# AlonKellner/hifi-gan

Measured on NVIDIA B200. Metric: V1 audio samples/sec, higher is better.
Workload: dtype bf16

## Files before the change

### hifi-gan_b200/csrc/hg_common.cuh

```cuda
#pragma once

#include <cuda_runtime.h>
#include <cuda_bf16.h>
#include <cuda.h>
#include <stdint.h>
#include <stdio.h>

#define HG_OK 0
#define HG_ERR_INVALID (-1)
#define HG_ERR_CUDA (-2)
#define HG_ERR_UNSUPPORTED (-3)
#define HG_ERR_DRIVER (-4)

void hg_set_error(const char* fmt, ...);

#define HG_CHECK_CUDA(expr)                                                        \
  do {                                                                             \
    cudaError_t _e = (expr);                                                       \
    if (_e != cudaSuccess) {                                                       \
      hg_set_error("%s:%d: %s -> %s", __FILE__, __LINE__, #expr,                   \
                   cudaGetErrorString(_e));                                        \
      return HG_ERR_CUDA;                                                          \
    }                                                                              \
  } while (0)
// ... 54 lines not shown
      "selp.b32 %0, 1, 0, P;\n\t"
      "}\n"
      : "=r"(ok)
      : "r"(smem_u32(bar)), "r"(parity)
      : "memory");
  return ok != 0;
}
__device__ __forceinline__ void mbar_wait(uint64_t* bar, uint32_t parity) {
  uint32_t spins = 0;
  while (!mbar_try_wait(bar, parity)) {
    if (++spins > HG_SPIN_LIMIT) {
      printf("hg: mbarrier wait timed out (block %d thread %d)\n", (int)blockIdx.x, (int)threadIdx.x);
      __trap();
    }
  }
}

__device__ __forceinline__ void tma_prefetch_desc(const CUtensorMap* m) {
  asm volatile("prefetch.tensormap [%0];" ::"l"(reinterpret_cast<uint64_t>(m)) : "memory");
}
__device__ __forceinline__ void tma_load_3d(void* smem_dst, const CUtensorMap* m, uint64_t* bar,
                                            int32_t c0, int32_t c1, int32_t c2) {
  asm volatile(
      "cp.async.bulk.tensor.3d.shared::cluster.global.mbarrier::complete_tx::bytes"
      " [%0], [%1, {%3, %4, %5}], [%2];"
      :
      : "r"(smem_u32(smem_dst)), "l"(reinterpret_cast<uint64_t>(m)), "r"(smem_u32(bar)), "r"(c0),
        "r"(c1), "r"(c2)
      : "memory");
}

__device__ __forceinline__ void tc_fence_before() {
  asm volatile("tcgen05.fence::before_thread_sync;" ::: "memory");
}
__device__ __forceinline__ void tc_fence_after() {
  asm volatile("tcgen05.fence::after_thread_sync;" ::: "memory");
}
__device__ __forceinline__ void tmem_alloc(uint32_t* smem_result, uint32_t ncols) {
  asm volatile("tcgen05.alloc.cta_group::1.sync.aligned.shared::cta.b32 [%0], %1;" ::"r"(
                   smem_u32(smem_result)),
               "r"(ncols)
               : "memory");
  asm volatile("tcgen05.relinquish_alloc_permit.cta_group::1.sync.aligned;" ::: "memory");
}
__device__ __forceinline__ void tmem_dealloc(uint32_t taddr, uint32_t ncols) {
  asm volatile("tcgen05.dealloc.cta_group::1.sync.aligned.b32 %0, %1;" ::"r"(taddr), "r"(ncols)
               : "memory");
}
__device__ __forceinline__ void umma_bf16_ss_lo(uint32_t d_tmem, uint32_t a_lo, uint32_t b_lo,
                                                uint32_t desc_hi, uint32_t idesc, uint32_t accumulate) {
  asm volatile(
      "{\n\t"
      ".reg .pred p;\n\t"
      ".reg .b64 da, db;\n\t"
      "setp.ne.b32 p, %5, 0;\n\t"
      "mov.b64 da, {%1, %3};\n\t"
      "mov.b64 db, {%2, %3};\n\t"
      "tcgen05.mma.cta_group::1.kind::f16 [%0], da, db, %4, p;\n\t"
      "}\n"
      :
      : "r"(d_tmem), "r"(a_lo), "r"(b_lo), "r"(desc_hi), "r"(idesc), "r"(accumulate)
      : "memory");
}
__device__ __forceinline__ uint32_t cluster_ctarank() {
  uint32_t r;
  asm volatile("mov.u32 %0, %%cluster_ctarank;" : "=r"(r));
  return r;
}
__device__ __forceinline__ void cluster_sync_all() {
  asm volatile("barrier.cluster.arrive.release.aligned;" ::: "memory");
  asm volatile("barrier.cluster.wait.acquire.aligned;" ::: "memory");
}
__device__ __forceinline__ void mbar_arrive_remote(uint64_t* bar, uint32_t cta) {
  asm volatile(
      "{\n\t"
      ".reg .b32 remAddr32;\n\t"
      "mapa.shared::cluster.u32 remAddr32, %0, %1;\n\t"
      "mbarrier.arrive.shared::cluster.b64 _, [remAddr32];\n\t"
      "}\n"
      :
      : "r"(smem_u32(bar)), "r"(cta)
      : "memory");
}
__device__ __forceinline__ void tma_load_3d_2sm(void* smem_dst, const CUtensorMap* m, uint64_t* bar,
                                                int32_t c0, int32_t c1, int32_t c2) {
  asm volatile(
      "cp.async.bulk.tensor.3d.cta_group::2.shared::cluster.global.mbarrier::complete_tx::bytes"
      " [%0], [%1, {%3, %4, %5}], [%2];"
      :
      : "r"(smem_u32(smem_dst)), "l"(reinterpret_cast<uint64_t>(m)), "r"(smem_u32(bar) & 0xFEFFFFFFu),
        "r"(c0), "r"(c1), "r"(c2)
      : "memory");
}
__device__ __forceinline__ void tmem_alloc_2sm(uint32_t* smem_result, uint32_t ncols) {
  asm volatile("tcgen05.alloc.cta_group::2.sync.aligned.shared::cta.b32 [%0], %1;" ::"r"(
                   smem_u32(smem_result)),
               "r"(ncols)
               : "memory");
  asm volatile("tcgen05.relinquish_alloc_permit.cta_group::2.sync.aligned;" ::: "memory");
}
__device__ __forceinline__ void tmem_dealloc_2sm(uint32_t taddr, uint32_t ncols) {
  asm volatile("tcgen05.dealloc.cta_group::2.sync.aligned.b32 %0, %1;" ::"r"(taddr), "r"(ncols)
               : "memory");
}
__device__ __forceinline__ void umma_bf16_ss_lo_2sm(uint32_t d_tmem, uint32_t a_lo, uint32_t b_lo,
                                                    uint32_t desc_hi, uint32_t idesc, uint32_t accumulate) {
  asm volatile(
      "{\n\t"
      ".reg .pred p;\n\t"
      ".reg .b64 da, db;\n\t"
      "setp.ne.b32 p, %5, 0;\n\t"
      "mov.b64 da, {%1, %3};\n\t"
      "mov.b64 db, {%2, %3};\n\t"
      "tcgen05.mma.cta_group::2.kind::f16 [%0], da, db, %4, p;\n\t"
      "}\n"
      :
      : "r"(d_tmem), "r"(a_lo), "r"(b_lo), "r"(desc_hi), "r"(idesc), "r"(accumulate)
      : "memory");
}
__device__ __forceinline__ void umma_commit_2sm(uint64_t* bar) {
  asm volatile(
      "tcgen05.commit.cta_group::2.mbarrier::arrive::one.shared::cluster.multicast::cluster.b64 [%0], %1;"
      :
      : "r"(smem_u32(bar)), "h"(static_cast<uint16_t>(3))
      : "memory");
}

__device__ __forceinline__ uint32_t umma_desc_lo(uint32_t saddr) {
  return ((saddr & 0x3FFFFu) >> 4) | (1u << 16);
}
__device__ __forceinline__ uint32_t umma_desc_hi(uint32_t sbo_bytes, uint32_t layout_type) {
  return ((sbo_bytes >> 4) & 0x3FFFu) | (1u << 14) | ((layout_type & 7u) << 29);
}
__device__ __forceinline__ void umma_commit(uint64_t* bar) {
  asm volatile("tcgen05.commit.cta_group::1.mbarrier::arrive::one.shared::cluster.b64 [%0];" ::"r"(
                   smem_u32(bar))
               : "memory");
}
__device__ __forceinline__ void tmem_ld_wait() {
  asm volatile("tcgen05.wait::ld.sync.aligned;" ::: "memory");
}


__host__ __device__ constexpr uint32_t umma_idesc_bf16(uint32_t M, uint32_t N) {
  return (1u << 4) | (1u << 7) | (1u << 10) | ((N >> 3) << 17) | ((M >> 4) << 24);
}

__device__ __forceinline__ float lrelu(float v, float slope) { return v > 0.f ? v : v * slope; }

__device__ __forceinline__ uint32_t pack_bf16x2(float lo, float hi) {
  __nv_bfloat162 h = __floats2bfloat162_rn(lo, hi);
  return *reinterpret_cast<uint32_t*>(&h);
}
__device__ __forceinline__ float2 unpack_bf16x2(uint32_t w) {
  __nv_bfloat162 h = *reinterpret_cast<__nv_bfloat162*>(&w);
  return __bfloat1622float2(h);
}

struct U8 {
  uint32_t v[8];
};

__device__ __forceinline__ U8 ldg256(const void* p) {
  U8 r;
  asm volatile("ld.global.nc.L1::no_allocate.v8.b32 {%0,%1,%2,%3,%4,%5,%6,%7}, [%8];"
               : "=r"(r.v[0]), "=r"(r.v[1]), "=r"(r.v[2]), "=r"(r.v[3]), "=r"(r.v[4]), "=r"(r.v[5]),
// ... 77 lines not shown
```

### hifi-gan_b200/csrc/hg_resblock_pair.cu

```cuda
#include "hg_common.cuh"

#include <atomic>

#include "../../include/hifigan_b200.h"

extern std::atomic<int64_t> g_hg_launches;

namespace {

constexpr int kM = 128;
constexpr int kXformWarps = 4;
__host__ __device__ constexpr int epi_halves(int c) { return c == 64 ? 2 : 1; }
__host__ __device__ constexpr int pair_threads(int c) { return 64 + (kXformWarps + 8 * epi_halves(c)) * 32; }
constexpr int kMaxXSlots = 4;

struct PairArgs {
  int batch, t, c;
  int ktaps, dil1;
  int single;
  int subs;
  int r_out;
  int pad1, pad2;
  int a_rows;
  int x_boxes, x_box_rows;
// ... 291 lines not shown
      }
      int i = 0, m = 0;
      for (int u = 0; u < n_units; ++u) {
        const uint32_t a = i & 1u, ph = (i >> 1) & 1u;
        off = off_next; valid = valid_next; keep = keep_next;
#pragma unroll
        for (int g = 0; g < kG; ++g) rcur[g] = rnext[g];
        if (u + 1 < n_units) {
          off_next = next_unit_off(valid_next, keep_next);
          if (valid_next) {
#pragma unroll
            for (int g = 0; g < kG; ++g) rnext[g] = hg::ldg256(p.x + off_next + g * 16);
          }
        }
        constexpr bool kPreRes = kMrf && (C == 32);
        hg::U8 r1[kPreRes ? kG : 1], r2[kPreRes ? kG : 1];
        if (kPreRes && valid && p.res1) {
#pragma unroll
          for (int g = 0; g < kG; ++g) r1[kPreRes ? g : 0] = hg::ldg256(p.res1 + off + g * 16);
        }
        if (kPreRes && valid && p.res2) {
#pragma unroll
          for (int g = 0; g < kG; ++g) r2[kPreRes ? g : 0] = hg::ldg256(p.res2 + off + g * 16);
        }
        if (m == 0) {
          hg::mbar_wait(&full_bar[a], ph);
          hg::tc_fence_after();
        }
#pragma unroll
        for (int g = 0; g < kG; ++g) {
          uint32_t raw[16];
          hg::tmem_ld_32x16(tmem_base + lane_base + acc_base + a * acc_cols + m * C + col0 + g * 16, raw);
          hg::tmem_ld_wait();
          if (g == kG - 1 && m == S - 1) {
            hg::tc_fence_before();
            __syncwarp();
            if (lane == 0) hg::mbar_arrive(&empty_bar[a]);
          }
          if (valid) {
            float v[16];
#pragma unroll
            for (int q = 0; q < 4; ++q) {
              const float4 bq = *reinterpret_cast<const float4*>(bias + col0 + g * 16 + 4 * q);
              v[4 * q] = __uint_as_float(raw[4 * q]) + bq.x;
              v[4 * q + 1] = __uint_as_float(raw[4 * q + 1]) + bq.y;
              v[4 * q + 2] = __uint_as_float(raw[4 * q + 2]) + bq.z;
              v[4 * q + 3] = __uint_as_float(raw[4 * q + 3]) + bq.w;
            }
            if (kActIn) hg::add_bf16x16_unlrelu(v, rcur[g], p.x_inv);
            else hg::add_bf16x16(v, rcur[g]);
            if (kMrf && p.res1) hg::add_bf16x16(v, kPreRes ? r1[kPreRes ? g : 0] : hg::ldg256(p.res1 + off + g * 16));
            if (kMrf && p.res2) hg::add_bf16x16(v, kPreRes ? r2[kPreRes ? g : 0] : hg::ldg256(p.res2 + off + g * 16));
            if (kMrf) {
              const float sc = keep ? p.scale : 0.f;
#pragma unroll
              for (int e = 0; e < 16; ++e) v[e] *= sc;
            }
            if (p.out_raw) {
              hg::U8 o;
#pragma unroll
              for (int q = 0; q < 8; ++q) o.v[q] = hg::pack_bf16x2(v[2 * q], v[2 * q + 1]);
              hg::stg256(p.out_raw + off + g * 16, o);
            }
            if (kMrf && p.out_act) {
              hg::U8 o;
#pragma unroll
              for (int q = 0; q < 8; ++q)
                o.v[q] = hg::pack_bf16x2(hg::lrelu(v[2 * q], p.out_slope), hg::lrelu(v[2 * q + 1], p.out_slope));
              hg::stg256(p.out_act + off + g * 16, o);
            }
          }
        }
        if (++m == S) { m = 0; ++i; }
      }
    }
  }

  hg::tc_fence_before();
  __syncthreads();
  hg::tc_fence_after();
  if (warp == 1) hg::tmem_dealloc(tmem_base, tmem_cols);
}

int g_sms = 0, g_smem = 0;

template <int C, bool kSingle, bool kMrf, bool kActIn>
int launch_pair_as(const CUtensorMap& tx, const CUtensorMap& tw1, const CUtensorMap& tw2, const PairArgs& p,
                size_t smem_bytes, int grid, cudaStream_t st) {
  static hg::PerDeviceOnce once;
  if (once.need())
    HG_CHECK_CUDA(cudaFuncSetAttribute(resblock_pair_kernel<C, kSingle, kMrf, kActIn>,
                                       cudaFuncAttributeMaxDynamicSharedMemorySize, g_smem));
  resblock_pair_kernel<C, kSingle, kMrf, kActIn><<<grid, pair_threads(C), smem_bytes, st>>>(tx, tw1, tw2, p);
  HG_CHECK_CUDA(cudaGetLastError());
  return HG_OK;
}

template <int C, bool kSingle>
int launch_pair(const CUtensorMap& tx, const CUtensorMap& tw1, const CUtensorMap& tw2, const PairArgs& p,
                bool act_in, size_t smem_bytes, int grid, cudaStream_t st) {
  const bool mrf = p.res1 || p.res2 || p.out_act || p.item_len || p.scale != 1.f;
  if (act_in)
    return mrf ? launch_pair_as<C, kSingle, true, true>(tx, tw1, tw2, p, smem_bytes, grid, st)
               : launch_pair_as<C, kSingle, false, true>(tx, tw1, tw2, p, smem_bytes, grid, st);
  return mrf ? launch_pair_as<C, kSingle, true, false>(tx, tw1, tw2, p, smem_bytes, grid, st)
             : launch_pair_as<C, kSingle, false, false>(tx, tw1, tw2, p, smem_bytes, grid, st);
}

size_t pair_smem_bytes(int c, int ktaps, int dil1, int subs, int x_slots, int single, PairArgs* out) {
  const uint32_t row = static_cast<uint32_t>(c) * 2;
  const uint32_t a_rows = subs * kM + (ktaps - 1) * dil1;
  const uint32_t boxes = (a_rows + 255) / 256;
  const uint32_t box_rows = ((a_rows + boxes - 1) / boxes + 15) & ~15u;
  const uint32_t x_slot = (boxes * box_rows * row + 1023u) & ~1023u;
  const uint32_t t1_slot = single ? 0u : ((subs * kM + ktaps - 1) * row + 1023u) & ~1023u;
  const uint32_t w_bytes = static_cast<uint32_t>(ktaps) * c * row;
  if (box_rows > 256) return ~static_cast<size_t>(0);
  if (out) {
    out->subs = subs; out->a_rows = a_rows; out->x_boxes = boxes; out->x_box_rows = box_rows;
    out->x_slot_bytes = x_slot; out->t1_slot_bytes = t1_slot; out->w_bytes = w_bytes;
  }
  return 1024 + static_cast<size_t>(x_slots) * x_slot + 2 * static_cast<size_t>(t1_slot) +
         (single ? 1 : 2) * static_cast<size_t>(w_bytes) + sizeof(PairBarriers);
}

int pick_subs(int c, int ktaps, int dil1, int single) {
  for (int subs = 512 / (4 * c); subs >= 1; subs >>= 1)
    if (pair_smem_bytes(c, ktaps, dil1, subs, 2, single, nullptr) <= static_cast<size_t>(g_smem)) return subs;
  return 0;
}

}

extern "C" int hg_resblock_pair_supported(int c, int ktaps, int dil1) {
  if (!(c == 32 || c == 64) || ktaps < 1 || !(ktaps & 1) || dil1 < 1) return 0;
  if (kM + (ktaps - 1) * dil1 > 256 || ktaps > 65) return 0;
  if (!g_smem) {
    int dev = 0;
    if (cudaGetDevice(&dev) != cudaSuccess) return 0;
    cudaDeviceGetAttribute(&g_sms, cudaDevAttrMultiProcessorCount, dev);
    cudaDeviceGetAttribute(&g_smem, cudaDevAttrMaxSharedMemoryPerBlockOptin, dev);
  }
  return pick_subs(c, ktaps, dil1, 0) > 0 ? 1 : 0;
}

extern "C" int hg_resblock_single_supported(int c, int ktaps, int dil1) {
  if (!hg_resblock_pair_supported(c, 1, 1) && !g_smem) return 0;
  if (!(c == 32 || c == 64) || ktaps < 1 || !(ktaps & 1) || dil1 < 1 || ktaps > 65) return 0;
  return pick_subs(c, ktaps, dil1, 1) > 0 ? 1 : 0;
}

namespace {

int resblock_pair_fwd(const void* x, bool act_in, const void* w1_packed, const float* b1, const void* w2_packed,
                      const float* b2, int batch, int t, int c, int ktaps, int dil1, float in_slope, const void* res1,
                      const void* res2, float scale, void* out_raw, void* out_act, float out_slope,
                      const int* item_len, int item_mul, void* stream) {
  const int single = w2_packed == nullptr;
  HG_REQUIRE(x && w1_packed && b1 && (single || b2), "hg_resblock_pair_fwd: null input");
  HG_REQUIRE(out_raw || out_act, "hg_resblock_pair_fwd: no output requested");
  HG_REQUIRE(batch > 0 && t > 0, "hg_resblock_pair_fwd: empty batch/time");
  HG_REQUIRE(hg_resblock_pair_supported(c, ktaps, dil1) || (single && hg_resblock_single_supported(c, ktaps, dil1)),
             "hg_resblock_pair_fwd: unsupported shape c=%d k=%d d=%d (use hg_conv1d_fwd)", c, ktaps, dil1);
  PairArgs p{};
  p.batch = batch; p.t = t; p.c = c; p.ktaps = ktaps; p.dil1 = dil1;
  const int subs = pick_subs(c, ktaps, dil1, single);
  p.single = single;
  p.r_out = single ? subs * kM : subs * kM + 1 - ktaps;
  p.pad1 = (ktaps - 1) * dil1 / 2;
  p.pad2 = single ? 0 : (ktaps - 1) / 2;
  p.tiles_t = (t + p.r_out - 1) / p.r_out;
  p.num_tiles = batch * p.tiles_t;
  int slots = kMaxXSlots;
  while (slots > 2 && pair_smem_bytes(c, ktaps, dil1, subs, slots, single, nullptr) > static_cast<size_t>(g_smem)) --slots;
  p.x_slots = slots;
  const size_t smem_bytes = pair_smem_bytes(c, ktaps, dil1, subs, slots, single, &p);
  p.x = static_cast<const __nv_bfloat16*>(x);
  p.b1 = b1; p.b2 = single ? b1 : b2;
  p.res1 = static_cast<const __nv_bfloat16*>(res1);
  p.res2 = static_cast<const __nv_bfloat16*>(res2);
  p.scale = scale; p.in_slope = in_slope; p.out_slope = out_slope;
  p.out_raw = static_cast<__nv_bfloat16*>(out_raw);
  p.out_act = static_cast<__nv_bfloat16*>(out_act);
  p.item_len = item_len; p.item_mul = item_mul > 0 ? item_mul : 1;
  p.x_inv = act_in ? 1.f / in_slope : 1.f;

  CUtensorMap tx, tw1, tw2;
  const int swz = c * 2;
  int rc = hg_encode_tmap_bf16_3d(&tx, x, c, t, batch, static_cast<uint64_t>(c) * 2,
                                  static_cast<uint64_t>(t) * c * 2, c, p.x_box_rows, 1, swz);
  if (rc) return rc;
  rc = hg_encode_tmap_bf16_3d(&tw1, w1_packed, c, c, ktaps, static_cast<uint64_t>(c) * 2,
                              static_cast<uint64_t>(c) * c * 2, c, c, ktaps, swz);
  if (rc) return rc;
  rc = hg_encode_tmap_bf16_3d(&tw2, single ? w1_packed : w2_packed, c, c, ktaps, static_cast<uint64_t>(c) * 2,
                              static_cast<uint64_t>(c) * c * 2, c, c, ktaps, swz);
  if (rc) return rc;
  const int grid = p.num_tiles < g_sms ? p.num_tiles : g_sms;
  cudaStream_t st = static_cast<cudaStream_t>(stream);
  if (single)
    rc = (c == 64) ? launch_pair<64, true>(tx, tw1, tw2, p, act_in, smem_bytes, grid, st)
                   : launch_pair<32, true>(tx, tw1, tw2, p, act_in, smem_bytes, grid, st);
  else
    rc = (c == 64) ? launch_pair<64, false>(tx, tw1, tw2, p, act_in, smem_bytes, grid, st)
                   : launch_pair<32, false>(tx, tw1, tw2, p, act_in, smem_bytes, grid, st);
  if (rc) return rc;
  g_hg_launches.fetch_add(1, std::memory_order_relaxed);
  return HG_OK;
}

}

extern "C" int hg_resblock_pair_fwd(const void* x, const void* w1_packed, const float* b1,
                                    const void* w2_packed, const float* b2, int batch, int t, int c,
                                    int ktaps, int dil1, float in_slope, const void* res1,
                                    const void* res2, float scale, void* out_raw, void* out_act,
                                    float out_slope, const int* item_len, int item_mul, void* stream) {
  return resblock_pair_fwd(x, false, w1_packed, b1, w2_packed, b2, batch, t, c, ktaps, dil1, in_slope, res1, res2,
                           scale, out_raw, out_act, out_slope, item_len, item_mul, stream);
}

extern "C" int hg_resblock_pair_fwd_actin(const void* x_act, const void* w1_packed, const float* b1,
                                          const void* w2_packed, const float* b2, int batch, int t, int c,
                                          int ktaps, int dil1, float in_slope, const void* res1,
                                          const void* res2, float scale, void* out_raw, void* out_act,
                                          float out_slope, const int* item_len, int item_mul, void* stream) {
  HG_REQUIRE(in_slope > 0.f && in_slope <= 1.f, "hg_resblock_pair_fwd_actin: slope %g not in (0, 1]", in_slope);
  return resblock_pair_fwd(x_act, true, w1_packed, b1, w2_packed, b2, batch, t, c, ktaps, dil1, in_slope, res1, res2,
                           scale, out_raw, out_act, out_slope, item_len, item_mul, stream);
}
```

### hifi-gan_b200/models.py

```python
from __future__ import annotations

import os
import warnings
from ctypes import byref, c_int
from typing import Dict, List, Optional, Tuple

import torch
import torch.nn as nn
from torch.nn import AvgPool1d, Conv1d, Conv2d, ConvTranspose1d
from torch.nn.utils import remove_weight_norm, spectral_norm, weight_norm

from . import _lib
from .utils import get_padding, init_weights

LRELU_SLOPE = 0.1


def _wn(module: nn.Module) -> nn.Module:
    with warnings.catch_warnings():
        warnings.simplefilter("ignore")
        return weight_norm(module)


def _pad_ch(c: int) -> int:
# ... 96 lines not shown
                if g is not None:
                    g = torch.cat([g, g.new_zeros(self.cout_p - self.cout)], 0)
            v = v.contiguous()
            _lib.check(L.hg_pack_conv1d_weight(v.data_ptr(), 0 if g is None else g.contiguous().data_ptr(),
                                               self.cout_p, self.cin, self.taps, self.cin_p,
                                               self.w.data_ptr(), _stream()), "hg_pack_conv1d_weight")
            if b is not None and self.cout_p == self.cout and b.is_contiguous():
                self.bias = b
            else:
                self.bias.zero_()
                if b is not None:
                    self.bias[: self.cout].copy_(b)
        else:
            k = m.kernel_size[0]
            if self.cout_p != self.cout or self.cin_p != self.cin:
                vp = v.new_zeros(self.cin_p, self.cout_p, k)
                vp[: self.cin, : self.cout] = v
                v = vp
                if g is not None:
                    g = torch.cat([g, g.new_zeros(self.cin_p - self.cin)], 0)
            v = v.contiguous()
            _lib.check(L.hg_pack_convtr1d_weight(v.data_ptr(), 0 if g is None else g.contiguous().data_ptr(),
                                                 self.cin_p, self.cout_p, k, self.stride, m.padding[0],
                                                 self.w.data_ptr(), _stream()), "hg_pack_convtr1d_weight")
            self.bias.zero_()
            if b is not None:
                self.bias.view(self.stride, self.cout_p)[:, : self.cout].copy_(b.unsqueeze(0).expand(self.stride, -1))
        self.key = key


def _conv(L, x, pc: _PackedConv, batch: int, t: int, *, res=(None, None, None), res0_slope=0.0, scale=1.0,
          out_raw=None, out_act=None, slope=LRELU_SLOPE, item=(0, 1)) -> None:
    p = [0 if r is None else r.data_ptr() for r in res]
    outs = (0 if out_raw is None else out_raw.data_ptr(), 0 if out_act is None else out_act.data_ptr(), slope,
            item[0], item[1], _stream())
    head = (x.data_ptr(), pc.w.data_ptr(), pc.bias.data_ptr(), batch, t, pc.cin_p, pc.w.shape[1], pc.taps, pc.dil,
            pc.pad_left)
    if res0_slope:
        _lib.check(L.hg_conv1d_fwd_actres(*head, p[0], res0_slope, p[1], p[2], scale, *outs), "hg_conv1d_fwd_actres")
    else:
        _lib.check(L.hg_conv1d_fwd(*head, p[0], p[1], p[2], scale, *outs), "hg_conv1d_fwd")


def _pair(L, x, pc1: _PackedConv, pc2: _PackedConv, batch: int, t: int, *, x_act=False, res=(None, None),
          scale=1.0, out_raw=None, out_act=None, slope=LRELU_SLOPE, item=(0, 1)) -> None:
    p = [0 if r is None else r.data_ptr() for r in res]
    w2, b2 = (0, 0) if pc2 is None else (pc2.w.data_ptr(), pc2.bias.data_ptr())
    fn, name = ((L.hg_resblock_pair_fwd_actin, "hg_resblock_pair_fwd_actin") if x_act
                else (L.hg_resblock_pair_fwd, "hg_resblock_pair_fwd"))
    _lib.check(fn(x.data_ptr(), pc1.w.data_ptr(), pc1.bias.data_ptr(), w2, b2, batch, t, pc1.cin_p, pc1.taps,
                  pc1.dil, LRELU_SLOPE, p[0], p[1], scale, 0 if out_raw is None else out_raw.data_ptr(),
                  0 if out_act is None else out_act.data_ptr(), slope, item[0], item[1], _stream()), name)


_FUSE_PAIRS = True


def _pair_ok(L, pc1: _PackedConv, pc2: _PackedConv) -> bool:
    return bool(_FUSE_PAIRS and pc1.cin_p == pc1.cout_p == pc2.cin_p == pc2.cout_p and pc1.taps == pc2.taps
                and pc2.dil == 1 and L.hg_resblock_pair_supported(pc1.cin_p, pc1.taps, pc1.dil))


def _single_ok(L, pc: _PackedConv) -> bool:
    return bool(_FUSE_PAIRS and pc.cin_p == pc.cout_p and L.hg_resblock_single_supported(pc.cin_p, pc.taps, pc.dil))


def _block_plan(L, block: "nn.Module", packs: List[_PackedConv]) -> List[bool]:
    if not isinstance(block, ResBlock1):
        return [_single_ok(L, pc) for pc in packs]
    return [_pair_ok(L, packs[2 * i], packs[2 * i + 1]) for i in range(len(packs) // 2)]


def _resblock_chain(L, block: "nn.Module", packs: List[_PackedConv], batch: int, t: int, c_p: int,
                    x_raw, x_act, bufs: Dict[str, torch.Tensor], final, item=(0, 1)) -> None:
    two_conv = isinstance(block, ResBlock1)
    fused = _block_plan(L, block, packs)
    steps = len(fused)
    cur_raw, cur_act = x_raw, x_act
    ping = [(bufs["a_raw"], bufs["a_act"]), (bufs["b_raw"], bufs["b_act"])]
    for i in range(steps):
        last = i == steps - 1
        nr, na = ping[i & 1]
        if not last:
            nr, na = (nr, None) if fused[i + 1] else (None, na)
        if fused[i]:
            pc1, pc2 = (packs[2 * i], packs[2 * i + 1]) if two_conv else (packs[i], None)
            x, x_is_act = (cur_raw, False) if cur_raw is not None else (cur_act, True)
            if last:
                final(dict(pair=(pc1, pc2), x=x, x_act=x_is_act))
            else:
                _pair(L, x, pc1, pc2, batch, t, x_act=x_is_act, out_raw=nr, out_act=na, item=item)
        else:
            if two_conv:
                _conv(L, cur_act, packs[2 * i], batch, t, out_act=bufs["t1"], item=item)
                src, pc = bufs["t1"], packs[2 * i + 1]
            else:
                src, pc = cur_act, packs[i]
            res0, res0_slope = (cur_raw, 0.0) if cur_raw is not None else (cur_act, LRELU_SLOPE)
            if last:
                final(dict(pc=pc, x=src, res0=res0, res0_slope=res0_slope))
            else:
                _conv(L, src, pc, batch, t, res=(res0, None, None), res0_slope=res0_slope, out_raw=nr, out_act=na,
                      item=item)
        cur_raw, cur_act = nr, na


class _StandaloneBlockMixin:

    def _packs(self, device) -> List[_PackedConv]:
        cache = self.__dict__.setdefault("_hg_packs", None)
        convs = self._ordered_convs()
        if cache is None or cache[0].w.device != device:
            cache = [_PackedConv(m, "conv", device) for m in convs]
            self.__dict__["_hg_packs"] = cache
        for pc in cache:
            pc.refresh()
        return cache

    def forward(self, x: torch.Tensor) -> torch.Tensor:
        _require_cuda(x, type(self).__name__)
        if _wants_grad(x, self):
            raise NotImplementedError(f"{type(self).__name__} on its own is an inference surface (call it under "
                                      "torch.no_grad()); it is differentiable as part of Generator")
        L = _lib.lib()
        b, c, t = x.shape
        packs = self._packs(x.device)
        c_p = packs[0].cin_p
        mk = lambda: torch.empty(b, t, c_p, dtype=torch.bfloat16, device=x.device)
        bufs = {k: mk() for k in ("x_raw", "x_act", "t1", "a_raw", "a_act", "b_raw", "b_act", "out")}
        xin = x.contiguous().float()
        _lib.check(L.hg_ncl_to_nlc(xin.data_ptr(), b, c, t, c_p, bufs["x_raw"].data_ptr(),
                                   bufs["x_act"].data_ptr(), LRELU_SLOPE, _stream()), "hg_ncl_to_nlc")

        def final(kw):
            if "pair" in kw:
                _pair(L, kw["x"], *kw["pair"], b, t, x_act=kw["x_act"], out_raw=bufs["out"])
            else:
                _conv(L, kw["x"], kw["pc"], b, t, res=(kw["res0"], None, None), res0_slope=kw["res0_slope"],
                      out_raw=bufs["out"])

        _resblock_chain(L, self, packs, b, t, c_p, bufs["x_raw"], bufs["x_act"], bufs, final)
        y = torch.empty(b, c_p, t, dtype=torch.float32, device=x.device)
        _lib.check(L.hg_nlc_to_ncl(bufs["out"].data_ptr(), b, t, c_p, y.data_ptr(), _stream()), "hg_nlc_to_ncl")
        return y[:, :c].contiguous() if c_p != c else y


class ResBlock1(_StandaloneBlockMixin, torch.nn.Module):

    def __init__(self, h, channels, kernel_size=3, dilation=(1, 3, 5)):
        super().__init__()
        self.h = h

        def conv(d):
            return _wn(Conv1d(channels, channels, kernel_size, 1, dilation=d,
                              padding=get_padding(kernel_size, d)))

        self.convs1 = nn.ModuleList([conv(d) for d in dilation[:3]])
        self.convs1.apply(init_weights)
        self.convs2 = nn.ModuleList([conv(1) for _ in dilation[:3]])
        self.convs2.apply(init_weights)

    def _ordered_convs(self):
        out = []
        for c1, c2 in zip(self.convs1, self.convs2):
            out += [c1, c2]
        return out

# ... 458 lines not shown
```

Baseline: 344.7 million.

## Add 2-CTA cluster fused resblock pair kernel for 128 channels

Adds a new fused two-conv resblock kernel for 128-channel layers that runs across a 2-CTA cluster with cta_group::2 UMMA and shared TMEM. The intermediate activation stays in shared memory rather than going through global memory as a separate conv launch. The Python chain now passes activated inputs between 128-channel steps. The intent is to cut the global round trip and launch overhead of the 128-channel resblocks, at the cost of complex cluster synchronisation and a single t1 slot that may serialize the pipeline.

```diff
diff --git a/hifi-gan_b200/csrc/hg_common.cuh b/hifi-gan_b200/csrc/hg_common.cuh
--- a/hifi-gan_b200/csrc/hg_common.cuh
+++ b/hifi-gan_b200/csrc/hg_common.cuh
@@ -160,6 +160,37 @@
       : "r"(smem_u32(bar)), "r"(cta)
       : "memory");
 }
+__device__ __forceinline__ void mbar_arrive_release_cluster(uint64_t* bar, uint32_t cta) {
+  asm volatile(
+      "{\n\t"
+      ".reg .b32 remAddr32;\n\t"
+      "mapa.shared::cluster.u32 remAddr32, %0, %1;\n\t"
+      "mbarrier.arrive.release.cluster.shared::cluster.b64 _, [remAddr32];\n\t"
+      "}\n"
+      :
+      : "r"(smem_u32(bar)), "r"(cta)
+      : "memory");
+}
+__device__ __forceinline__ void mbar_wait_cluster(uint64_t* bar, uint32_t parity) {
+  uint32_t spins = 0;
+  for (;;) {
+    uint32_t ok;
+    asm volatile(
+        "{\n\t"
+        ".reg .pred P;\n\t"
+        "mbarrier.try_wait.parity.acquire.cluster.shared::cta.b64 P, [%1], %2;\n\t"
+        "selp.b32 %0, 1, 0, P;\n\t"
+        "}\n"
+        : "=r"(ok)
+        : "r"(smem_u32(bar)), "r"(parity)
+        : "memory");
+    if (ok) return;
+    if (++spins > HG_SPIN_LIMIT) {
+      printf("hg: mbarrier wait timed out (block %d thread %d)\n", (int)blockIdx.x, (int)threadIdx.x);
+      __trap();
+    }
+  }
+}
 __device__ __forceinline__ void tma_load_3d_2sm(void* smem_dst, const CUtensorMap* m, uint64_t* bar,
                                                 int32_t c0, int32_t c1, int32_t c2) {
   asm volatile(
diff --git a/hifi-gan_b200/csrc/hg_resblock_pair.cu b/hifi-gan_b200/csrc/hg_resblock_pair.cu
--- a/hifi-gan_b200/csrc/hg_resblock_pair.cu
+++ b/hifi-gan_b200/csrc/hg_resblock_pair.cu
@@ -397,6 +397,326 @@
   if (warp == 1) hg::tmem_dealloc(tmem_base, tmem_cols);
 }
 
+constexpr int kC2 = 128;
+constexpr uint32_t kC2ChunkRow = 128;
+constexpr uint32_t kC2WTap = 64 * kC2ChunkRow;
+constexpr int kC2RoleWarps = 8;
+__host__ __device__ constexpr int pair2_xform_warps(bool act_in) { return act_in ? 0 : 2; }
+__host__ __device__ constexpr int pair2_threads(bool act_in) {
+  return 64 + (pair2_xform_warps(act_in) + 2 * kC2RoleWarps) * 32;
+}
+#ifndef HG_PAIR128_T1_SLOTS
+#define HG_PAIR128_T1_SLOTS 1
+#endif
+constexpr int kC2T1Slots = HG_PAIR128_T1_SLOTS;
+constexpr int kC2XSlots = 3 - kC2T1Slots;
+
+struct Pair2Barriers {
+  uint64_t x_full[2], x_ready[2], x_empty[2];
+  uint64_t w_full;
+  uint64_t acc1_full[2], acc1_empty[2], t1_full[2], t1_empty[2], acc2_full[2], acc2_empty[2];
+  uint32_t tmem_base;
+  uint32_t pad;
+  __align__(16) float b1[kC2];
+  __align__(16) float b2[kC2];
+};
+
+template <bool kMrf, bool kActIn>
+__global__ void __cluster_dims__(2, 1, 1) __launch_bounds__(pair2_threads(kActIn), 1)
+resblock_pair2_kernel(const __grid_constant__ CUtensorMap tm_x, const __grid_constant__ CUtensorMap tm_w1,
+                      const __grid_constant__ CUtensorMap tm_w2, const PairArgs p) {
+  constexpr int kXform = pair2_xform_warps(kActIn);
+  constexpr uint32_t kSbo = 8 * kC2ChunkRow;
+  constexpr int kG = 4;
+  extern __shared__ uint8_t smem_raw[];
+  uint8_t* smem = reinterpret_cast<uint8_t*>((reinterpret_cast<uintptr_t>(smem_raw) + 1023) &
+                                             ~static_cast<uintptr_t>(1023));
+  uint8_t* x_buf = smem;
+  uint8_t* t1_buf = x_buf + kC2XSlots * p.x_slot_bytes;
+  uint8_t* w1_buf = t1_buf + kC2T1Slots * p.t1_slot_bytes;
+  uint8_t* w2_buf = w1_buf + p.w_bytes;
+  Pair2Barriers* bars = reinterpret_cast<Pair2Barriers*>(w2_buf + p.w_bytes);
+  const uint32_t x_chunk = static_cast<uint32_t>(p.x_box_rows) * kC2ChunkRow;
+  const uint32_t t1_chunk = p.t1_slot_bytes / 2;
+  const uint32_t w_chunk = p.w_bytes / 2;
+
+  const int warp = threadIdx.x >> 5;
+  const int lane = threadIdx.x & 31;
+  const uint32_t rank = hg::cluster_ctarank();
+  const int n_clusters = static_cast<int>(gridDim.x) >> 1;
+  const int cluster_id = static_cast<int>(blockIdx.x) >> 1;
+  const int n_local = (p.num_tiles - cluster_id + n_clusters - 1) / n_clusters;
+  const int pt_step = n_clusters % p.tiles_t, b_step = n_clusters / p.tiles_t;
+
+  if (warp == 0 && lane == 0) {
+    hg::tma_prefetch_desc(&tm_x);
+    hg::tma_prefetch_desc(&tm_w1);
+    hg::tma_prefetch_desc(&tm_w2);
+  }
+  if (warp == 1) {
+    if (lane == 0) {
+      for (int i = 0; i < 2; ++i) {
+        hg::mbar_init(&bars->x_full[i], kActIn ? 2 : 1);
+        hg::mbar_init(&bars->x_ready[i], kActIn ? 1 : 2 * kXform);
+        hg::mbar_init(&bars->x_empty[i], 1);
+        hg::mbar_init(&bars->acc1_full[i], 1);
+        hg::mbar_init(&bars->acc1_empty[i], 2 * kC2RoleWarps);
+        hg::mbar_init(&bars->t1_full[i], 2 * kC2RoleWarps);
+        hg::mbar_init(&bars->t1_empty[i], 1);
+        hg::mbar_init(&bars->acc2_full[i], 1);
+        hg::mbar_init(&bars->acc2_empty[i], 2 * kC2RoleWarps);
+      }
+      hg::mbar_init(&bars->w_full, 2);
+      hg::fence_mbar_init();
+    }
+    __syncwarp();
+    hg::tmem_alloc_2sm(&bars->tmem_base, 512);
+  }
+  if (threadIdx.x < kC2) {
+    bars->b1[threadIdx.x] = p.b1[threadIdx.x];
+    bars->b2[threadIdx.x] = p.b2[threadIdx.x];
+  }
+  for (uint32_t i = threadIdx.x * 16; i < kC2T1Slots * p.t1_slot_bytes; i += pair2_threads(kActIn) * 16)
+    *reinterpret_cast<uint4*>(t1_buf + i) = make_uint4(0, 0, 0, 0);
+  hg::fence_proxy_async_smem();
+  hg::tc_fence_before();
+  __syncthreads();
+  hg::cluster_sync_all();
+  hg::tc_fence_after();
+  const uint32_t tmem_base = *reinterpret_cast<volatile uint32_t*>(&bars->tmem_base);
+
+  if (warp == 0) {
+    if (lane == 0) {
+      if (rank == 0) hg::mbar_arrive_expect_tx(&bars->w_full, 4 * p.w_bytes);
+      else hg::mbar_arrive_remote(&bars->w_full, 0);
+      for (int c = 0; c < 2; ++c) {
+        hg::tma_load_3d_2sm(w1_buf + c * w_chunk, &tm_w1, &bars->w_full, c * 64, static_cast<int>(rank) * 64, 0);
+        hg::tma_load_3d_2sm(w2_buf + c * w_chunk, &tm_w2, &bars->w_full, c * 64, static_cast<int>(rank) * 64, 0);
+      }
+      int pt = cluster_id % p.tiles_t, b = cluster_id / p.tiles_t;
+      uint32_t slot = 0, phase = 0;
+      for (int i = 0; i < n_local; ++i) {
+        hg::mbar_wait(&bars->x_empty[slot], phase ^ 1u);
+        const int row0 = (2 * pt + static_cast<int>(rank)) * p.r_out - p.pad2 - p.pad1;
+        uint8_t* dst = x_buf + slot * p.x_slot_bytes;
+        if (kActIn) {
+          if (rank == 0) hg::mbar_arrive_expect_tx(&bars->x_full[slot], 2 * p.x_slot_bytes);
+          else hg::mbar_arrive_remote(&bars->x_full[slot], 0);
+          for (int c = 0; c < 2; ++c) hg::tma_load_3d_2sm(dst + c * x_chunk, &tm_x, &bars->x_full[slot], c * 64, row0, b);
+        } else {
+          hg::mbar_arrive_expect_tx(&bars->x_full[slot], p.x_slot_bytes);
+          for (int c = 0; c < 2; ++c) hg::tma_load_3d(dst + c * x_chunk, &tm_x, &bars->x_full[slot], c * 64, row0, b);
+        }
+        if (++slot == kC2XSlots) { slot = 0; phase ^= 1u; }
+        pt += pt_step; b += b_step;
+        if (pt >= p.tiles_t) { pt -= p.tiles_t; ++b; }
+      }
+    }
+    __syncwarp();
+  } else if (warp == 1) {
+    if (rank == 0) {
+      constexpr uint32_t idesc = hg::umma_idesc_bf16(2 * kM, kC2);
+      const uint32_t desc_hi = hg::umma_desc_hi(kSbo, 2u);
+      const uint32_t w1_lo = hg::umma_desc_lo(hg::smem_u32(w1_buf));
+      const uint32_t w2_lo = hg::umma_desc_lo(hg::smem_u32(w2_buf));
+      const uint32_t x_tap_step = static_cast<uint32_t>(p.dil1) * (kC2ChunkRow >> 4);
+      hg::mbar_wait_cluster(&bars->w_full, 0);
+      hg::tc_fence_after();
+      auto issue = [&](uint32_t d, uint32_t a_lo, uint32_t a_chunk, uint32_t w_lo, uint32_t a_step) {
+        uint32_t accumulate = 0;
+        for (int c = 0; c < 2; ++c) {
+          uint32_t al = a_lo + c * (a_chunk >> 4), wl = w_lo + c * (w_chunk >> 4);
+          for (int j = 0; j < p.ktaps; ++j) {
+#pragma unroll
+            for (int kk = 0; kk < 4; ++kk) {
+              hg::umma_bf16_ss_lo_2sm(d, al + kk * 2, wl + kk * 2, desc_hi, idesc, accumulate);
+              accumulate = 1;
+            }
+            al += a_step;
+            wl += kC2WTap >> 4;
+          }
+        }
+      };
+      uint32_t x_slot = 0, x_phase = 0, t_slot = 0, t_phase = 0;
+      auto conv1 = [&](int i) {
+        const uint32_t slot = x_slot, a = i & 1u, ph = (i >> 1) & 1u;
+        hg::mbar_wait_cluster(kActIn ? &bars->x_full[slot] : &bars->x_ready[slot], x_phase);
+        if (++x_slot == kC2XSlots) { x_slot = 0; x_phase ^= 1u; }
+        hg::mbar_wait_cluster(&bars->acc1_empty[a], ph ^ 1u);
+        hg::tc_fence_after();
+        if (hg::elect_one()) {
+          issue(tmem_base + a * kC2, hg::umma_desc_lo(hg::smem_u32(x_buf + slot * p.x_slot_bytes)), x_chunk, w1_lo,
+                x_tap_step);
+          hg::umma_commit_2sm(&bars->x_empty[slot]);
+          hg::umma_commit_2sm(&bars->acc1_full[a]);
+        }
+        __syncwarp();
+      };
+      auto conv2 = [&](int i) {
+        const uint32_t slot = t_slot, a = i & 1u, ph = (i >> 1) & 1u;
+        hg::mbar_wait_cluster(&bars->t1_full[slot], t_phase);
+        if (++t_slot == kC2T1Slots) { t_slot = 0; t_phase ^= 1u; }
+        hg::mbar_wait_cluster(&bars->acc2_empty[a], ph ^ 1u);
+        hg::tc_fence_after();
+        if (hg::elect_one()) {
+          issue(tmem_base + 2 * kC2 + a * kC2, hg::umma_desc_lo(hg::smem_u32(t1_buf + slot * p.t1_slot_bytes)),
+                t1_chunk, w2_lo, kC2ChunkRow >> 4);
+          hg::umma_commit_2sm(&bars->t1_empty[slot]);
+          hg::umma_commit_2sm(&bars->acc2_full[a]);
+        }
+        __syncwarp();
+      };
+      if (n_local > 0) conv1(0);
+      for (int i = 0; i < n_local; ++i) {
+        if (i + 1 < n_local) conv1(i + 1);
+        conv2(i);
+      }
+    }
+  } else if (warp < 2 + kXform) {
+    const int tid = (warp - 2) * 32 + lane;
+    const __nv_bfloat162 slope2 = __float2bfloat162_rn(p.in_slope);
+    const int n_chunks = p.a_rows * static_cast<int>(kC2ChunkRow / 16);
+    uint32_t slot = 0, phase = 0;
+    for (int i = 0; i < n_local; ++i) {
+      hg::mbar_wait(&bars->x_full[slot], phase);
+      for (int c = 0; c < 2; ++c) {
+        uint4* xs = reinterpret_cast<uint4*>(x_buf + slot * p.x_slot_bytes + c * x_chunk);
+        for (int q = tid; q < n_chunks; q += kXform * 32) {
+          uint4 v = xs[q];
+          v.x = lrelu_bf16x2(v.x, slope2); v.y = lrelu_bf16x2(v.y, slope2);
+          v.z = lrelu_bf16x2(v.z, slope2); v.w = lrelu_bf16x2(v.w, slope2);
+          xs[q] = v;
+        }
+      }
+      hg::fence_proxy_async_smem();
+      __syncwarp();
+      if (lane == 0) hg::mbar_arrive_release_cluster(&bars->x_ready[slot], 0);
+      if (++slot == kC2XSlots) { slot = 0; phase ^= 1u; }
+    }
+  } else {
+    const int ew = warp - (2 + kXform);
+    const int quarter = warp & 3;
+    const int half = (ew >> 2) & 1;
+    const int row = quarter * 32 + lane;
+    const uint32_t lane_base = static_cast<uint32_t>(quarter * 32) << 16;
+    const int col0 = half * 64;
+    int pt = cluster_id % p.tiles_t, bb = cluster_id / p.tiles_t;
+
+    if (ew < kC2RoleWarps) {
+      const uint32_t swz = row & 7;
+      uint32_t slot = 0, phase = 0;
+      for (int i = 0; i < n_local; ++i) {
+        const uint32_t a = i & 1u, ph = (i >> 1) & 1u;
+        hg::mbar_wait(&bars->acc1_full[a], ph);
+        hg::mbar_wait(&bars->t1_empty[slot], phase ^ 1u);
+        hg::tc_fence_after();
+        const int t_item = (kMrf && p.item_len) ? min(p.t, __ldg(p.item_len + bb) * p.item_mul) : p.t;
+        const int time = (2 * pt + static_cast<int>(rank)) * p.r_out - p.pad2 + row;
+        const bool inside = time >= 0 && time < t_item;
+        uint8_t* trow = t1_buf + slot * p.t1_slot_bytes + half * t1_chunk + static_cast<uint32_t>(row) * kC2ChunkRow;
+#pragma unroll
+        for (int g = 0; g < kG; ++g) {
+          uint32_t raw[16];
+          hg::tmem_ld_32x16(tmem_base + lane_base + a * kC2 + col0 + g * 16, raw);
+          hg::tmem_ld_wait();
+          if (g == kG - 1) {
+            hg::tc_fence_before();
+            __syncwarp();
+            if (lane == 0) hg::mbar_arrive_release_cluster(&bars->acc1_empty[a], 0);
+          }
+          uint32_t o[8];
+#pragma unroll
+          for (int q = 0; q < 4; ++q) {
+            const float4 bq = *reinterpret_cast<const float4*>(bars->b1 + col0 + g * 16 + 4 * q);
+            const float v0 = hg::lrelu(__uint_as_float(raw[4 * q]) + bq.x, p.in_slope);
+            const float v1 = hg::lrelu(__uint_as_float(raw[4 * q + 1]) + bq.y, p.in_slope);
+            const float v2 = hg::lrelu(__uint_as_float(raw[4 * q + 2]) + bq.z, p.in_slope);
+            const float v3 = hg::lrelu(__uint_as_float(raw[4 * q + 3]) + bq.w, p.in_slope);
+            o[2 * q] = inside ? hg::pack_bf16x2(v0, v1) : 0u;
+            o[2 * q + 1] = inside ? hg::pack_bf16x2(v2, v3) : 0u;
+          }
+          const uint32_t chunk = g * 2;
+          *reinterpret_cast<uint4*>(trow + ((chunk ^ swz) << 4)) = make_uint4(o[0], o[1], o[2], o[3]);
+          *reinterpret_cast<uint4*>(trow + (((chunk + 1) ^ swz) << 4)) = make_uint4(o[4], o[5], o[6], o[7]);
+        }
+        hg::fence_proxy_async_smem();
+        __syncwarp();
+        if (lane == 0) hg::mbar_arrive_release_cluster(&bars->t1_full[slot], 0);
+        if (++slot == kC2T1Slots) { slot = 0; phase ^= 1u; }
+        pt += pt_step; bb += b_step;
+        if (pt >= p.tiles_t) { pt -= p.tiles_t; ++bb; }
+      }
+    } else {
+      for (int i = 0; i < n_local; ++i) {
+        const uint32_t a = i & 1u, ph = (i >> 1) & 1u;
+        const int time = (2 * pt + static_cast<int>(rank)) * p.r_out + row;
+        const bool valid = row < p.r_out && time < p.t;
+        const bool keep = !kMrf || !p.item_len || time < __ldg(p.item_len + bb) * p.item_mul;
+        const size_t off = (static_cast<size_t>(bb) * p.t + (valid ? time : 0)) * kC2 + col0;
+        hg::U8 rx[kG];
+        if (valid) {
+#pragma unroll
+          for (int g = 0; g < kG; ++g) rx[g] = hg::ldg256(p.x + off + g * 16);
+        }
+        hg::mbar_wait(&bars->acc2_full[a], ph);
+        hg::tc_fence_after();
+#pragma unroll
+        for (int g = 0; g < kG; ++g) {
+          uint32_t raw[16];
+          hg::tmem_ld_32x16(tmem_base + lane_base + 2 * kC2 + a * kC2 + col0 + g * 16, raw);
+          hg::tmem_ld_wait();
+          if (g == kG - 1) {
+            hg::tc_fence_before();
+            __syncwarp();
+            if (lane == 0) hg::mbar_arrive_release_cluster(&bars->acc2_empty[a], 0);
+          }
+          if (valid) {
+            float v[16];
+#pragma unroll
+            for (int q = 0; q < 4; ++q) {
+              const float4 bq = *reinterpret_cast<const float4*>(bars->b2 + col0 + g * 16 + 4 * q);
+              v[4 * q] = __uint_as_float(raw[4 * q]) + bq.x;
+              v[4 * q + 1] = __uint_as_float(raw[4 * q + 1]) + bq.y;
+              v[4 * q + 2] = __uint_as_float(raw[4 * q + 2]) + bq.z;
+              v[4 * q + 3] = __uint_as_float(raw[4 * q + 3]) + bq.w;
+            }
+            if (kActIn) hg::add_bf16x16_unlrelu(v, rx[g], p.x_inv);
+            else hg::add_bf16x16(v, rx[g]);
+            if (kMrf && p.res1) hg::add_bf16x16(v, hg::ldg256(p.res1 + off + g * 16));
+            if (kMrf && p.res2) hg::add_bf16x16(v, hg::ldg256(p.res2 + off + g * 16));
+            if (kMrf) {
+              const float sc = keep ? p.scale : 0.f;
+#pragma unroll
+              for (int e = 0; e < 16; ++e) v[e] *= sc;
+            }
+            if (p.out_raw) {
+              hg::U8 o;
+#pragma unroll
+              for (int q = 0; q < 8; ++q) o.v[q] = hg::pack_bf16x2(v[2 * q], v[2 * q + 1]);
+              hg::stg256(p.out_raw + off + g * 16, o);
+            }
+            if (p.out_act) {
+              hg::U8 o;
+#pragma unroll
+              for (int q = 0; q < 8; ++q)
+                o.v[q] = hg::pack_bf16x2(hg::lrelu(v[2 * q], p.out_slope), hg::lrelu(v[2 * q + 1], p.out_slope));
+              hg::stg256(p.out_act + off + g * 16, o);
+            }
+          }
+        }
+        pt += pt_step; bb += b_step;
+        if (pt >= p.tiles_t) { pt -= p.tiles_t; ++bb; }
+      }
+    }
+  }
+
+  hg::tc_fence_before();
+  __syncthreads();
+  hg::cluster_sync_all();
+  hg::tc_fence_after();
+  if (warp == 1) hg::tmem_dealloc_2sm(tmem_base, 512);
+}
+
 int g_sms = 0, g_smem = 0;
 
 template <int C, bool kSingle, bool kMrf, bool kActIn>
@@ -445,10 +765,25 @@
   return 0;
 }
 
+size_t pair2_smem_bytes(int ktaps, int dil1, PairArgs* out) {
+  const uint32_t a_rows = kM + (ktaps - 1) * dil1;
+  const uint32_t box_rows = (a_rows + 15) & ~15u;
+  const uint32_t x_slot = 2 * box_rows * kC2ChunkRow;
+  const uint32_t t1_slot = 2 * ((kM + ktaps - 1 + 7) & ~7u) * kC2ChunkRow;
+  const uint32_t w_bytes = static_cast<uint32_t>(ktaps) * 2 * kC2WTap;
+  if (box_rows > 256) return ~static_cast<size_t>(0);
+  if (out) {
+    out->subs = 1; out->a_rows = a_rows; out->x_boxes = 1; out->x_box_rows = box_rows; out->x_slots = kC2XSlots;
+    out->x_slot_bytes = x_slot; out->t1_slot_bytes = t1_slot; out->w_bytes = w_bytes;
+  }
+  return 1024 + static_cast<size_t>(kC2XSlots) * x_slot + static_cast<size_t>(kC2T1Slots) * t1_slot +
+         2 * static_cast<size_t>(w_bytes) + sizeof(Pair2Barriers);
+}
+
 }
 
 extern "C" int hg_resblock_pair_supported(int c, int ktaps, int dil1) {
-  if (!(c == 32 || c == 64) || ktaps < 1 || !(ktaps & 1) || dil1 < 1) return 0;
+  if (!(c == 32 || c == 64 || c == 128) || ktaps < 1 || !(ktaps & 1) || dil1 < 1) return 0;
   if (kM + (ktaps - 1) * dil1 > 256 || ktaps > 65) return 0;
   if (!g_smem) {
     int dev = 0;
@@ -456,6 +791,7 @@
     cudaDeviceGetAttribute(&g_sms, cudaDevAttrMultiProcessorCount, dev);
     cudaDeviceGetAttribute(&g_smem, cudaDevAttrMaxSharedMemoryPerBlockOptin, dev);
   }
+  if (c == 128) return g_sms >= 2 && pair2_smem_bytes(ktaps, dil1, nullptr) <= static_cast<size_t>(g_smem) ? 1 : 0;
   return pick_subs(c, ktaps, dil1, 0) > 0 ? 1 : 0;
 }
 
@@ -466,6 +802,62 @@
 }
 
 namespace {
+
+template <bool kMrf, bool kActIn>
+int launch_pair2_as(const CUtensorMap& tx, const CUtensorMap& tw1, const CUtensorMap& tw2, const PairArgs& p,
+                    size_t smem_bytes, int grid, cudaStream_t st) {
+  static hg::PerDeviceOnce once;
+  if (once.need())
+    HG_CHECK_CUDA(cudaFuncSetAttribute(resblock_pair2_kernel<kMrf, kActIn>,
+                                       cudaFuncAttributeMaxDynamicSharedMemorySize, g_smem));
+  resblock_pair2_kernel<kMrf, kActIn><<<grid, pair2_threads(kActIn), smem_bytes, st>>>(tx, tw1, tw2, p);
+  HG_CHECK_CUDA(cudaGetLastError());
+  return HG_OK;
+}
+
+int resblock_pair2_fwd(const void* x, bool act_in, const void* w1_packed, const float* b1, const void* w2_packed,
+                       const float* b2, int batch, int t, int ktaps, int dil1, float in_slope, const void* res1,
+                       const void* res2, float scale, void* out_raw, void* out_act, float out_slope,
+                       const int* item_len, int item_mul, void* stream) {
+  PairArgs p{};
+  p.batch = batch; p.t = t; p.c = kC2; p.ktaps = ktaps; p.dil1 = dil1;
+  p.r_out = kM + 1 - ktaps;
+  p.pad1 = (ktaps - 1) * dil1 / 2;
+  p.pad2 = (ktaps - 1) / 2;
+  p.tiles_t = (t + 2 * p.r_out - 1) / (2 * p.r_out);
+  p.num_tiles = batch * p.tiles_t;
+  const size_t smem_bytes = pair2_smem_bytes(ktaps, dil1, &p);
+  p.x = static_cast<const __nv_bfloat16*>(x);
+  p.b1 = b1; p.b2 = b2;
+  p.res1 = static_cast<const __nv_bfloat16*>(res1);
+  p.res2 = static_cast<const __nv_bfloat16*>(res2);
+  p.scale = scale; p.in_slope = in_slope; p.out_slope = out_slope;
+  p.out_raw = static_cast<__nv_bfloat16*>(out_raw);
+  p.out_act = static_cast<__nv_bfloat16*>(out_act);
+  p.item_len = item_len; p.item_mul = item_mul > 0 ? item_mul : 1;
+  p.x_inv = act_in ? 1.f / in_slope : 1.f;
+
+  CUtensorMap tx, tw1, tw2;
+  int rc = hg_encode_tmap_bf16_3d(&tx, x, kC2, t, batch, kC2 * 2, static_cast<uint64_t>(t) * kC2 * 2, 64,
+                                  p.x_box_rows, 1, 128);
+  if (rc) return rc;
+  rc = hg_encode_tmap_bf16_3d(&tw1, w1_packed, kC2, kC2, ktaps, kC2 * 2, kC2 * kC2 * 2, 64, 64, ktaps, 128);
+  if (rc) return rc;
+  rc = hg_encode_tmap_bf16_3d(&tw2, w2_packed, kC2, kC2, ktaps, kC2 * 2, kC2 * kC2 * 2, 64, 64, ktaps, 128);
+  if (rc) return rc;
+  const int grid = 2 * (p.num_tiles < g_sms / 2 ? p.num_tiles : g_sms / 2);
+  cudaStream_t st = static_cast<cudaStream_t>(stream);
+  const bool mrf = res1 || res2 || item_len || scale != 1.f;
+  if (act_in)
+    rc = mrf ? launch_pair2_as<true, true>(tx, tw1, tw2, p, smem_bytes, grid, st)
+             : launch_pair2_as<false, true>(tx, tw1, tw2, p, smem_bytes, grid, st);
+  else
+    rc = mrf ? launch_pair2_as<true, false>(tx, tw1, tw2, p, smem_bytes, grid, st)
+             : launch_pair2_as<false, false>(tx, tw1, tw2, p, smem_bytes, grid, st);
+  if (rc) return rc;
+  g_hg_launches.fetch_add(1, std::memory_order_relaxed);
+  return HG_OK;
+}
 
 int resblock_pair_fwd(const void* x, bool act_in, const void* w1_packed, const float* b1, const void* w2_packed,
                       const float* b2, int batch, int t, int c, int ktaps, int dil1, float in_slope, const void* res1,
@@ -475,8 +867,10 @@
   HG_REQUIRE(x && w1_packed && b1 && (single || b2), "hg_resblock_pair_fwd: null input");
   HG_REQUIRE(out_raw || out_act, "hg_resblock_pair_fwd: no output requested");
   HG_REQUIRE(batch > 0 && t > 0, "hg_resblock_pair_fwd: empty batch/time");
-  HG_REQUIRE(hg_resblock_pair_supported(c, ktaps, dil1) || (single && hg_resblock_single_supported(c, ktaps, dil1)),
+  HG_REQUIRE(single ? hg_resblock_single_supported(c, ktaps, dil1) : hg_resblock_pair_supported(c, ktaps, dil1),
              "hg_resblock_pair_fwd: unsupported shape c=%d k=%d d=%d (use hg_conv1d_fwd)", c, ktaps, dil1);
+  if (c == 128) return resblock_pair2_fwd(x, act_in, w1_packed, b1, w2_packed, b2, batch, t, ktaps, dil1, in_slope, res1,
+                                          res2, scale, out_raw, out_act, out_slope, item_len, item_mul, stream);
   PairArgs p{};
   p.batch = batch; p.t = t; p.c = c; p.ktaps = ktaps; p.dil1 = dil1;
   const int subs = pick_subs(c, ktaps, dil1, single);
diff --git a/hifi-gan_b200/models.py b/hifi-gan_b200/models.py
--- a/hifi-gan_b200/models.py
+++ b/hifi-gan_b200/models.py
@@ -202,7 +202,7 @@
         last = i == steps - 1
         nr, na = ping[i & 1]
         if not last:
-            nr, na = (nr, None) if fused[i + 1] else (None, na)
+            nr, na = (nr, None) if fused[i + 1] and c_p != 128 else (None, na)
         if fused[i]:
             pc1, pc2 = (packs[2 * i], packs[2 * i + 1]) if two_conv else (packs[i], None)
             x, x_is_act = (cur_raw, False) if cur_raw is not None else (cur_act, True)
```

Result: no change. 349.0 million, median of 6 (+1.2%).
